# MathsionYang/Ransac

Hardware: NVIDIA B200
Metric: hypothesis x point evaluations/s (useful, whole job); ms per robust fit in config (higher is better)
Workload: dtype f32

## Files before the change

ransac_b200/csrc/common.cuh:

```cuda
#pragma once
#include <cuda_runtime.h>
#include <stdint.h>

#include "../../include/usac_gpu.h"

#define USAC_REC_STRIDE 32
#define USAC_TILE_PAIRS 128
#ifndef USAC_WARP_STAGES
#define USAC_WARP_STAGES 2
#endif
#define USAC_SCORE_THREADS 128
#ifndef USAC_SCORE_MIN_CTAS
#define USAC_SCORE_MIN_CTAS 4
#endif
#ifndef USAC_SCORE_GRID_CTAS
#define USAC_SCORE_GRID_CTAS USAC_SCORE_MIN_CTAS
#endif
#ifndef USAC_SQ_MIN_CTAS
#define USAC_SQ_MIN_CTAS 5
#endif
#ifndef USAC_PPI
#define USAC_PPI 4
#endif

enum { REC_MODEL = 0, REC_HINV = 9, REC_BAND = 18, REC_THR = 22 };

struct ProblemDesc {
    int n;
    int n_pairs;
    long long aos_off;
    long long pair_off;
    float mx1, my1, mx2, my2;
    int neigh_type, knn;
    long long knn_off;
    long long grid_off;
    long long cell_start_off;
    long long growth_off, term_off, pool_off;
    long long cursor_off;
};

struct FitState {
    float best_model[9];
    int best_cnt;
// ... 57 lines not shown
```

ransac_b200/csrc/pipeline.cuh:

```cuda
#pragma once
#include "strict_math.cuh"

struct RoundArgs {
    const ProblemDesc* prob;
    const int* active;
    FitState* state;
    const float* aos;
    int est, K, S, m, mstride;
    int e5_all_roots;
    int midx_shift;
    int sampler, rng, neighbors;
    uint64_t seed;
    const int* table; unsigned table_rows;
    const unsigned* growth;
    const int* knn; const int* cell_of_point; const int* members; const int* rank_in_cell; const int* cell_start;
    unsigned* cursors;
    int* seeds;
    int* samples;
    float* models_raw;
    int* nmodels;
    int* offsets;
    float* recs;
    int* mvalid;
    uint2* items;
    unsigned* item_count;
    int* part_cnt; float* part_sum; int nchunks;
    uint2* sample_scores;
    float thr, confidence;
    unsigned max_iterations;
    const unsigned* term_tables;
    int rank, nranks;
    int sprt;
    const int* pool;
    struct SprtModelResult* sprt_res;
    int* done_out;
    unsigned before_sprt;
    int limit_remaining;
    void* const* peer_win;
    void* peer_self;
    unsigned peer_seq;
    unsigned peer_cap;
    unsigned* peer_counter;
    int* peer_error;
    unsigned long long hyp_base_p1;
};

#define USAC_PEER_HEADER_BYTES 1024
#define USAC_PEER_MAX_RANKS 64
// ... 339 lines not shown
}

__global__ void __launch_bounds__(1024) prepare_kernel(const RoundArgs a) {
    __shared__ int sm[33];
    const int slot = blockIdx.x;
    const int pid = a.active[slot];
    const ProblemDesc pd = a.prob[pid];
    const int per = (a.K + blockDim.x - 1) / blockDim.x;
    const int j0 = threadIdx.x * per, j1 = min(j0 + per, a.K);
    const int* nm = a.nmodels + (size_t)slot * a.K;
    int local = 0;
    for (int j = j0; j < j1; j++) local += nm[j];
    int total;
    int off = block_exclusive_scan(local, &total, sm);
    float rec[USAC_REC_STRIDE];
    for (int j = j0; j < j1; j++) {
        a.offsets[(size_t)slot * a.K + j] = off;
        const int k = nm[j];
        for (int i = 0; i < k; i++) {
            make_record(a.est, a.models_raw + (((size_t)slot * a.K + j) * a.S + i) * 9, a.thr, pd, rec);
            float4* dst = reinterpret_cast<float4*>(a.recs + ((size_t)slot * a.mstride + off + i) * USAC_REC_STRIDE);
#pragma unroll
            for (int w = 0; w < USAC_REC_STRIDE / 4; w++) dst[w] = make_float4(rec[4 * w], rec[4 * w + 1], rec[4 * w + 2], rec[4 * w + 3]);
        }
        off += k;
    }
    if (threadIdx.x == 0) a.mvalid[slot] = total;
    if (a.items) {
        __shared__ unsigned s_base;
        const unsigned ngroups = (unsigned)(total + 31) / 32u, count = ngroups * (unsigned)a.nchunks;
        if (threadIdx.x == 0) s_base = atomicAdd(a.item_count, count);
        __syncthreads();
        for (unsigned i = threadIdx.x; i < count; i += blockDim.x)
            a.items[s_base + i] = make_uint2((unsigned)slot, ((i / ngroups) << 16) | (i % ngroups));
    }
}

__device__ __forceinline__ bool score_bigger(int ca, float sa, int cb, float sb) {
    return ca > cb || (ca == cb && sa > sb);
}
__device__ __forceinline__ unsigned pack_cnt_midx(const RoundArgs& a, int cnt, int midx) { return (unsigned)cnt | ((unsigned)midx << a.midx_shift); }
__device__ __forceinline__ int packed_cnt(const RoundArgs& a, unsigned x) { return (int)(x & ((1u << a.midx_shift) - 1u)); }
__device__ __forceinline__ int packed_midx(const RoundArgs& a, unsigned x) { return (int)(x >> a.midx_shift); }
__device__ __forceinline__ int midx_none(const RoundArgs& a) { return (int)(0xffffffffu >> a.midx_shift); }

__global__ void reduce_kernel(const RoundArgs a) {
    const int slot = blockIdx.y, j = blockIdx.x * blockDim.x + threadIdx.x;
    if (j < a.K && !(a.nranks > 1 && (j % a.nranks) != a.rank)) {
        const int k = a.nmodels[(size_t)slot * a.K + j];
        const int off = a.offsets[(size_t)slot * a.K + j];
        int bc = -1, bi = 0;
        float bs = 0.f;
        for (int i = 0; i < k; i++) {
            int c = 0;
            float s = 0.f;
            for (int ch = 0; ch < a.nchunks; ch++) {
                const size_t o = ((size_t)slot * a.nchunks + ch) * a.mstride + off + i;
// ... 191 lines not shown
```

ransac_b200/csrc/score.cuh:

```cuda
#pragma once
#include "strict_math.cuh"

__device__ __forceinline__ float fast_rcp(float x) { float r; asm("rcp.approx.ftz.f32 %0, %1;" : "=f"(r) : "f"(x)); return r; }
__device__ __forceinline__ float fast_sqrt(float x) { float r; asm("sqrt.approx.ftz.f32 %0, %1;" : "=f"(r) : "f"(x)); return r; }
__device__ __forceinline__ float fast_rsqrt(float x) { float r; asm("rsqrt.approx.ftz.f32 %0, %1;" : "=f"(r) : "f"(x)); return r; }
__device__ __forceinline__ float2 dup(float x) { return make_float2(x, x); }

__device__ __forceinline__ uint32_t smem_u32(const void* p) { return (uint32_t)__cvta_generic_to_shared(p); }
__device__ __forceinline__ void mbar_init(uint64_t* bar, uint32_t count) {
    asm volatile("mbarrier.init.shared::cta.b64 [%0], %1;" ::"r"(smem_u32(bar)), "r"(count));
}
__device__ __forceinline__ void mbar_expect_tx(uint64_t* bar, uint32_t bytes) {
    asm volatile("mbarrier.arrive.expect_tx.shared::cta.b64 _, [%0], %1;" ::"r"(smem_u32(bar)), "r"(bytes) : "memory");
}
__device__ __forceinline__ bool mbar_try_wait(uint64_t* bar, uint32_t parity) {
    uint32_t ok;
    asm volatile(
        "{\n\t.reg .pred p;\n\t"
        "mbarrier.try_wait.parity.shared::cta.b64 p, [%1], %2;\n\t"
        "selp.u32 %0, 1, 0, p;\n\t}"
        : "=r"(ok)
        : "r"(smem_u32(bar)), "r"(parity)
        : "memory");
    return ok != 0;
// ... 237 lines not shown
        return make_float2(fabsf(v.x) + (negthr - band), fabsf(v.y) + (negthr - band));
    }
    __device__ __forceinline__ float reject_bound() const { return 0.f; }
    static __device__ __forceinline__ float finish(float sum_em, int cnt, float thr) { return sum_em + (float)cnt * thr; }
    static __device__ __forceinline__ float strict_to_em(float err, float thr) { return err - thr; }
};

struct ScoreArgs {
    const float* pairs;
    const float* aos;
    const ProblemDesc* prob;
    const int* active;
    const float* recs;
    const int* mvalid;
    int M, mstride;
    int chunk_pairs, nchunks;
    int mblocks, slots;
    int* part_cnt;
    float* part_sum;
    unsigned* work;
    unsigned work_base;
    const uint2* items;
    const unsigned* item_count;
};

__device__ __forceinline__ bool score_item(const ScoreArgs& a, unsigned item, unsigned total, int mgroups, int& slot, int& chunk, int& mgroup) {
    if (item >= total) return false;
    if (a.items) {
        const uint2 it = a.items[item];
        slot = (int)it.x; chunk = (int)(it.y >> 16); mgroup = (int)(it.y & 0xffffu);
    } else {
        mgroup = (int)(item % (unsigned)mgroups);
        const unsigned rest = item / (unsigned)mgroups;
        chunk = (int)(rest % (unsigned)a.nchunks); slot = (int)(rest / (unsigned)a.nchunks);
    }
    return true;
}

template <int EST>
__device__ __noinline__ float strict_em(const float* __restrict__ rec, const float* __restrict__ aos, int idx, int n) {
    if (idx >= n) return 0.f;
    const float thr = rec[REC_THR];
    float err;
    if (EST == USAC_EST_LINE2D) {
        const float2 p = reinterpret_cast<const float2*>(aos)[idx];
        err = strict_error<EST>(rec, p.x, p.y, 0.f, 0.f);
    } else {
        const float4 p = reinterpret_cast<const float4*>(aos)[idx];
        err = strict_error<EST>(rec, p.x, p.y, p.z, p.w);
    }
    return (err < thr) ? FastModel<EST>::strict_to_em(err, thr) : 0.f;
}

template <int EST>
__global__ void __launch_bounds__(USAC_SCORE_THREADS, USAC_SCORE_MIN_CTAS) score_kernel(const ScoreArgs a) {
    constexpr int PAIR_FLOATS = (EST == USAC_EST_LINE2D) ? 4 : 8;
    constexpr int NWARPS = USAC_SCORE_THREADS / 32;
    __shared__ __align__(128) float tile_all[NWARPS][USAC_WARP_STAGES][USAC_TILE_PAIRS * PAIR_FLOATS];
    __shared__ __align__(8) uint64_t full_all[NWARPS][USAC_WARP_STAGES];

    const int lane = threadIdx.x & 31, warp = threadIdx.x >> 5;
    float (*tile)[USAC_TILE_PAIRS * PAIR_FLOATS] = tile_all[warp];
    uint64_t* full = full_all[warp];
    if (lane == 0) {
#pragma unroll
        for (int s = 0; s < USAC_WARP_STAGES; s++) mbar_init(&full[s], 1);
        asm volatile("fence.mbarrier_init.release.cluster;" ::: "memory");
        asm volatile("fence.proxy.async.shared::cta;" ::: "memory");
    }
    __syncwarp();

    const int mgroups = a.mblocks * NWARPS;
    const unsigned total = a.items ? *a.item_count : (unsigned)a.slots * (unsigned)a.nchunks * (unsigned)mgroups;
    uint32_t g = 0;

    for (;;) {
        unsigned item = 0;
        if (lane == 0) item = atomicAdd(a.work, 1u) - a.work_base;
        item = __shfl_sync(0xffffffffu, item, 0);
        int slot, chunk, mgroup;
        if (!score_item(a, item, total, mgroups, slot, chunk, mgroup)) break;
        const int M = a.mvalid ? a.mvalid[slot] : a.M;
        if (mgroup * 32 >= M) continue;
        const ProblemDesc pd = a.prob[a.active ? a.active[slot] : slot];
        const int m = mgroup * 32 + lane;
        const bool live = m < M;
        const float* rec = a.recs + ((size_t)slot * a.mstride + (live ? m : 0)) * USAC_REC_STRIDE;
        const size_t out = ((size_t)slot * a.nchunks + chunk) * a.mstride + m;

        const int pair_begin = chunk * a.chunk_pairs;
        const int npairs = min(pair_begin + a.chunk_pairs, pd.n_pairs) - pair_begin;
        if (npairs <= 0) {
            if (live) { a.part_cnt[out] = 0; a.part_sum[out] = 0.f; }
            continue;
        }
        const int ntiles = (npairs + USAC_TILE_PAIRS - 1) / USAC_TILE_PAIRS;
        const float* src = a.pairs + ((size_t)pd.pair_off + pair_begin) * PAIR_FLOATS;

        if (lane == 0) {
            asm volatile("fence.proxy.async.shared::cta;" ::: "memory");
            for (int k = 0; k < USAC_WARP_STAGES && k < ntiles; k++) {
                const int s = (g + k) % USAC_WARP_STAGES;
                const uint32_t bytes = min(USAC_TILE_PAIRS, npairs - k * USAC_TILE_PAIRS) * PAIR_FLOATS * 4;
                mbar_expect_tx(&full[s], bytes);
// ... 256 lines not shown
```

ransac_b200/csrc/score_sq.cuh:

```cuda
#pragma once
#include "score.cuh"

#ifndef USAC_SQ_TRIPVOTE
#define USAC_SQ_TRIPVOTE 2
#endif
#ifndef USAC_SQ_PREFETCH
#define USAC_SQ_PREFETCH 0
#endif
#define USAC_SQ_LANE_CAP 16
#define USAC_SQ_FIXED_BITS 36
#define USAC_SQ_LO_BITS 22

__device__ __forceinline__ void sq_push(bool pred, uint32_t& qaddr, uint32_t entry) {
    asm volatile(
        "{\n\t.reg .pred p;\n\t"
        "setp.ne.u32 p, %1, 0;\n\t"
        "@p st.shared.u32 [%0], %2;\n\t"
        "@p add.u32 %0, %0, 128;\n\t}"
        : "+r"(qaddr)
        : "r"((uint32_t)pred), "r"(entry));
}

template <int EST>
__device__ __noinline__ void sq_drain(const uint32_t* __restrict__ q, uint32_t cnt, uint32_t* pre, const float* __restrict__ recs_group,
                                      const float* __restrict__ aos, int n, double scale, uint32_t* mcnt, uint32_t* mlo, uint32_t* mhi) {
    const int lane = threadIdx.x & 31;
    uint32_t incl = cnt;
#pragma unroll
    for (int o = 1; o < 32; o <<= 1) { const uint32_t y = __shfl_up_sync(0xffffffffu, incl, o); if (lane >= o) incl += y; }
    const uint32_t total = __shfl_sync(0xffffffffu, incl, 31);
    pre[lane] = incl - cnt;
    __syncwarp();
    for (uint32_t base = 0; base < total; base += 64) {
        int l[2], idx[2];
        bool on[2];
        float4 p[2];
#pragma unroll
        for (int h = 0; h < 2; h++) {
            const uint32_t t = base + 32u * h + lane;
            on[h] = t < total;
            l[h] = 0; idx[h] = 0;
            if (on[h]) {
                int ll = 0;
#pragma unroll
                for (int step = 16; step; step >>= 1) if (pre[ll + step] <= t) ll += step;
                l[h] = ll;
                idx[h] = (int)q[(t - pre[ll]) * 32 + ll];
                on[h] = idx[h] < n;
            }
            p[h] = make_float4(0.f, 0.f, 0.f, 0.f);
            if (on[h]) {
                if (EST == USAC_EST_LINE2D) { const float2 v = reinterpret_cast<const float2*>(aos)[idx[h]]; p[h] = make_float4(v.x, v.y, 0.f, 0.f); }
                else p[h] = reinterpret_cast<const float4*>(aos)[idx[h]];
            }
        }
#pragma unroll
        for (int h = 0; h < 2; h++) {
            if (!on[h]) continue;
            const float* rec = recs_group + (size_t)l[h] * USAC_REC_STRIDE;
            const float err = strict_error<EST>(rec, p[h].x, p[h].y, p[h].z, p[h].w);
            if (err < rec[REC_THR]) {
                const unsigned long long fix = __double2ull_rn((double)err * scale);
                atomicAdd(&mcnt[l[h]], 1u);
                atomicAdd(&mlo[l[h]], (uint32_t)(fix & ((1u << USAC_SQ_LO_BITS) - 1u)));
                atomicAdd(&mhi[l[h]], (uint32_t)(fix >> USAC_SQ_LO_BITS));
            }
        }
    }
}

template <int EST>
__global__ void __launch_bounds__(USAC_SCORE_THREADS, USAC_SQ_MIN_CTAS) score_sq_kernel(const ScoreArgs a) {
    constexpr int PAIR_FLOATS = (EST == USAC_EST_LINE2D) ? 4 : 8;
    constexpr int NWARPS = USAC_SCORE_THREADS / 32;
    static_assert(USAC_SQ_LANE_CAP >= 4 * USAC_PPI, "a lane's queue must hold two trips of pushes");
    __shared__ __align__(128) float tile_all[NWARPS][USAC_WARP_STAGES][USAC_TILE_PAIRS * PAIR_FLOATS];
    __shared__ __align__(8) uint64_t full_all[NWARPS][USAC_WARP_STAGES];
    __shared__ __align__(128) uint32_t queue_all[NWARPS][USAC_SQ_LANE_CAP * 32];
    __shared__ uint32_t macc_all[NWARPS][4][32];

    const int lane = threadIdx.x & 31, warp = threadIdx.x >> 5;
    float (*tile)[USAC_TILE_PAIRS * PAIR_FLOATS] = tile_all[warp];
    uint64_t* full = full_all[warp];
    uint32_t* queue = queue_all[warp];
    uint32_t* mcnt = macc_all[warp][0];
    uint32_t* mlo = macc_all[warp][1];
    uint32_t* mhi = macc_all[warp][2];
    uint32_t* pre = macc_all[warp][3];
    const uint32_t q_first = smem_u32(queue) + 4u * (uint32_t)lane;
    const uint32_t q_limit = q_first + 128u * (USAC_SQ_LANE_CAP - 2 * USAC_PPI);
    if (lane == 0) {
#pragma unroll
        for (int s = 0; s < USAC_WARP_STAGES; s++) mbar_init(&full[s], 1);
        asm volatile("fence.mbarrier_init.release.cluster;" ::: "memory");
        asm volatile("fence.proxy.async.shared::cta;" ::: "memory");
    }
    __syncwarp();

    const int mgroups = a.mblocks * NWARPS;
    const unsigned total = a.items ? *a.item_count : (unsigned)a.slots * (unsigned)a.nchunks * (unsigned)mgroups;
    uint32_t g = 0;

    unsigned pending = 0;
    if (USAC_SQ_PREFETCH && lane == 0) pending = atomicAdd(a.work, 1u) - a.work_base;
    for (;;) {
        if (!USAC_SQ_PREFETCH && lane == 0) pending = atomicAdd(a.work, 1u) - a.work_base;
        const unsigned item = __shfl_sync(0xffffffffu, pending, 0);
        int slot, chunk, mgroup;
        if (!score_item(a, item, total, mgroups, slot, chunk, mgroup)) break;
        if (USAC_SQ_PREFETCH && lane == 0) pending = atomicAdd(a.work, 1u) - a.work_base;
        const int M = a.mvalid ? a.mvalid[slot] : a.M;
        if (mgroup * 32 >= M) continue;
        const ProblemDesc pd = a.prob[a.active ? a.active[slot] : slot];
        const int m = mgroup * 32 + lane;
        const bool live = m < M;
        const float* recs_group = a.recs + ((size_t)slot * a.mstride + (size_t)mgroup * 32) * USAC_REC_STRIDE;
        const float* rec = recs_group + (size_t)(live ? lane : 0) * USAC_REC_STRIDE;
        const size_t out = ((size_t)slot * a.nchunks + chunk) * a.mstride + m;

        const int pair_begin = chunk * a.chunk_pairs;
        const int npairs = min(pair_begin + a.chunk_pairs, pd.n_pairs) - pair_begin;
        if (npairs <= 0) {
            if (live) { a.part_cnt[out] = 0; a.part_sum[out] = 0.f; }
            continue;
        }
        const int ntiles = (npairs + USAC_TILE_PAIRS - 1) / USAC_TILE_PAIRS;
        const float* src = a.pairs + ((size_t)pd.pair_off + pair_begin) * PAIR_FLOATS;

        if (lane == 0) {
            asm volatile("fence.proxy.async.shared::cta;" ::: "memory");
            for (int k = 0; k < USAC_WARP_STAGES && k < ntiles; k++) {
                const int s = (g + k) % USAC_WARP_STAGES;
                const uint32_t bytes = min(USAC_TILE_PAIRS, npairs - k * USAC_TILE_PAIRS) * PAIR_FLOATS * 4;
                mbar_expect_tx(&full[s], bytes);
                bulk_copy_g2s(tile[s], src + (size_t)k * USAC_TILE_PAIRS * PAIR_FLOATS, bytes, &full[s]);
            }
        }
        mcnt[lane] = 0u; mlo[lane] = 0u; mhi[lane] = 0u;
        uint32_t acc_cnt = 0;
        unsigned long long acc_sum = 0;
        __syncwarp();

        FastModel<EST> fm;
        fm.load(rec);
        const float thr = rec[REC_THR];
        const double scale = (double)(1ull << USAC_SQ_FIXED_BITS) / (double)thr;
// ... 55 lines not shown
                        load_pair(j + q, A, B);
                        const float2 z = fm.reject(A, B);
                        sq_push(!(z.x > zb) && live, qaddr, ebase + 2 * q);
                        sq_push(!(z.y > zb) && live, qaddr, ebase + 2 * q + 1);
                    }
                }
                if (__any_sync(0xffffffffu, qaddr > q_limit)) drain();
            }
            __syncwarp();
            if (lane == 0 && k + USAC_WARP_STAGES < ntiles) {
                asm volatile("fence.proxy.async.shared::cta;" ::: "memory");
                const int nk = k + USAC_WARP_STAGES;
                const uint32_t bytes = min(USAC_TILE_PAIRS, npairs - nk * USAC_TILE_PAIRS) * PAIR_FLOATS * 4;
                mbar_expect_tx(&full[s], bytes);
                bulk_copy_g2s(tile[s], src + (size_t)nk * USAC_TILE_PAIRS * PAIR_FLOATS, bytes, &full[s]);
            }
        }
        g += (uint32_t)ntiles;
        if (__any_sync(0xffffffffu, qaddr != q_first)) drain();
        if (live) {
            a.part_cnt[out] = (int)acc_cnt;
            a.part_sum[out] = (float)((double)acc_sum / scale);
        }
        __syncwarp();
    }
}
```

ransac_b200/csrc/usac_gpu.cu:

```cuda
#include <dlfcn.h>

#include <cub/device/device_radix_sort.cuh>
#include <cub/device/device_scan.cuh>

#include <algorithm>
#include <chrono>
#include <cmath>
#include <cstdio>
#include <cstdlib>
#include <cstring>
#include <map>
#include <string>
#include <thread>
#include <tuple>
#include <vector>

#include "essential.cuh"
#include "pipeline.cuh"
#include "score.cuh"
#include "score_sq.cuh"
#include "sprt.cuh"
#include "refit.cuh"
#include "lo.cuh"
#include "knn.cuh"
// ... 67 lines not shown
    DevBuf<unsigned> d_sprt_count;
    cudaStream_t stream2 = nullptr;
    cudaEvent_t ev_block[2] = {nullptr, nullptr};
    cudaEvent_t ev_round = nullptr;
    DevBuf<int> d_lo_bwave;
    DevBuf<LoSpec> d_lo_spec;
    DevBuf<LoWaveState> d_lo_ws;
    PinnedBuf<LoWaveState> h_lo_ws;
    DevBuf<unsigned> d_inl_ballots;
    DevBuf<int> d_inl_counts;
    PinnedBuf<int> h_rp_nmodels;
    PinnedBuf<SprtModelResult> h_rp_res;
    PinnedBuf<int2> h_rp_scores;
    PinnedBuf<float> h_rp_models;
    PinnedBuf<FitState> h_rp_state;
    DevBuf<int2> d_model_scores;
    DevBuf<float> d_pool_pts;
    DevBuf<unsigned long long> d_grid_keys;
    DevBuf<int> d_grid_ints;
    DevBuf<unsigned char> d_grid_temp;
    DevBuf<unsigned> d_work;
    DevBuf<uint2> d_items;
    DevBuf<unsigned> d_item_count;
    unsigned work_next = 0;
    DevBuf<int> d_knn_cells;
    DevBuf<float4> d_knn_pts;
    DevBuf<float> d_q_models, d_q_recs, d_q_sum, d_q_err;
    DevBuf<int> d_q_cnt, d_q_ids, d_q_ids2, d_q_ok, d_lo_ids_a, d_lo_ids_b, d_lo_small;
    DevBuf<float> d_q_model2;
    DevBuf<LoIO> d_lo_io;
    usac_allgather_fn allgather = nullptr;
    void* allgather_user = nullptr;
    void* nccl_lib = nullptr;
    void* nccl_comm = nullptr;
    void* peer_self = nullptr;
    unsigned peer_cap = 0;
    std::vector<void*> peer_opened;
    DevBuf<void*> d_peer_win;
    DevBuf<unsigned> d_peer_counter;
    DevBuf<int> d_peer_error;
    int* h_peer_error = nullptr;
    int peer_rank = -1, peer_nranks = 0;
    unsigned peer_seq = 0;
    unsigned long long peer_rounds = 0;
    std::map<std::tuple<int, int, float, unsigned>, std::vector<unsigned>> term_cache;
    std::vector<long long> term_signature;
// ... 68 lines not shown
}

extern "C" void usac_gpu_destroy(usac_gpu_ctx* c) {
    if (!c) return;
    cudaSetDevice(c->device);
    cudaStreamSynchronize(c->stream);
    if (c->stream2) cudaStreamDestroy(c->stream2);
    for (int i = 0; i < 2; i++) if (c->ev_block[i]) cudaEventDestroy(c->ev_block[i]);
    if (c->ev_round) cudaEventDestroy(c->ev_round);
    for (void* w : c->peer_opened) cudaIpcCloseMemHandle(w);
    if (c->peer_self) cudaFree(c->peer_self);
    if (c->h_peer_error) cudaFreeHost(c->h_peer_error);
    c->d_peer_win.release(); c->d_peer_counter.release(); c->d_peer_error.release();
    if (c->nccl_comm && c->nccl_lib) {
        typedef int (*destroy_fn)(void*);
        destroy_fn f = (destroy_fn)dlsym(c->nccl_lib, "ncclCommDestroy");
        if (f) f(c->nccl_comm);
    }
    c->d_aos.release(); c->d_pairs.release(); c->d_prob.release(); c->d_pair_offs.release(); c->d_state.release(); c->d_active.release(); c->d_active2.release(); c->d_state_init.release();
    c->d_knn.release(); c->d_cell_of_point.release(); c->d_members.release(); c->d_rank.release(); c->d_cell_start.release();
    c->d_pool.release(); c->d_cursors.release(); c->d_growth.release(); c->d_term.release();
    c->d_samples.release(); c->d_nmodels.release(); c->d_offsets.release(); c->d_mvalid.release(); c->d_part_cnt.release();
    c->d_seeds.release(); c->d_table.release(); c->d_models_raw.release(); c->d_recs.release(); c->d_part_sum.release();
    c->d_scores.release(); c->d_scores_all.release(); c->d_sprt_res.release(); c->d_sprt_carry.release(); c->d_sprt_count.release(); c->d_inl_ballots.release(); c->d_inl_counts.release(); c->d_lo_bwave.release(); c->d_lo_spec.release(); c->d_lo_ws.release(); c->h_lo_ws.release(); c->h_rp_nmodels.release(); c->h_rp_res.release(); c->h_rp_scores.release(); c->h_rp_models.release(); c->h_rp_state.release(); c->d_model_scores.release(); c->d_pool_pts.release(); c->d_grid_keys.release(); c->d_grid_ints.release(); c->d_grid_temp.release(); c->d_knn_cells.release(); c->d_knn_pts.release(); c->d_work.release(); c->d_items.release(); c->d_item_count.release();
    c->d_q_models.release(); c->d_q_recs.release(); c->d_q_sum.release(); c->d_q_err.release(); c->d_q_cnt.release(); c->d_q_ids.release(); c->d_q_ids2.release(); c->d_q_ok.release(); c->d_q_model2.release(); c->d_lo_ids_a.release(); c->d_lo_ids_b.release(); c->d_lo_small.release(); c->d_lo_io.release();
    if (c->h_state) cudaFreeHost(c->h_state);
    if (c->h_active) cudaFreeHost(c->h_active);
    if (c->h_done) cudaFreeHost(c->h_done);
    c->d_done.release();
    for (auto& pr : c->score_events) { cudaEventDestroy(pr.first); cudaEventDestroy(pr.second); }
    cudaEventDestroy(c->ev0); cudaEventDestroy(c->ev1);
    if (c->own_stream) cudaStreamDestroy(c->stream);
    delete c;
}

extern "C" int usac_gpu_set_stream(usac_gpu_ctx* c, void* cuda_stream) {
    if (!c) return USAC_ERR_ARG;
    cudaSetDevice(c->device);
    CUDA_TRY(c, cudaStreamSynchronize(c->stream));
    if (c->own_stream) cudaStreamDestroy(c->stream);
    c->stream = (cudaStream_t)cuda_stream;
    c->own_stream = false;
    return USAC_OK;
}

extern "C" const char* usac_gpu_last_error(const usac_gpu_ctx* c) { return c ? c->err.c_str() : g_create_error.c_str(); }

// ... 360 lines not shown
    u.grid += (size_t)n;
    u.cell_start += (size_t)n + 1;
    if (d.cursor_off < 0) CUDA_TRY(c, append_segment(c->d_cursors, u.cursors, (const unsigned*)nullptr, 3 * (size_t)n + 1, &d.cursor_off, c->stream));
    d.neigh_type = USAC_NEIGH_GRID;
    return push_desc(c);
}

extern "C" int usac_gpu_set_sprt_pool(usac_gpu_ctx* c, int problem, const int* pool) {
    if (!c || problem < 0 || problem >= c->P || !pool) return fail(c, USAC_ERR_ARG, "set_sprt_pool: bad arguments");
    cudaSetDevice(c->device);
    SideUsed& u = c->side;
    ProblemDesc& d = c->h_prob[problem];
    for (int i = 0; i < d.n; i++) if (pool[i] < 0 || pool[i] >= d.n) return fail(c, USAC_ERR_ARG, "set_sprt_pool: index out of range");
    CUDA_TRY(c, append_segment(c->d_pool, u.pool, pool, (size_t)d.n, &d.pool_off, c->stream));
    const int dim = usac_point_dim(c->est);
    CUDA_TRY(c, c->d_pool_pts.ensure((size_t)c->total_points * dim));
    pool_gather_kernel<<<(d.n + 255) / 256, 256, 0, c->stream>>>(c->d_aos.p + (size_t)d.aos_off * dim, c->d_pool.p + d.pool_off, d.n, dim,
                                                                  c->d_pool_pts.p + (size_t)d.aos_off * dim);
    CUDA_TRY(c, cudaGetLastError());
    c->h_pool_set[problem] = 1;
    return push_desc(c);
}

static void launch_score(usac_gpu_ctx* c, ScoreArgs a, int slots, int mblocks, bool dense_survivors = false) {
    a.mblocks = mblocks; a.slots = slots;
    constexpr int warps_per_cta = USAC_SCORE_THREADS / 32;
    const long long items = (long long)slots * a.nchunks * mblocks * warps_per_cta;
    const unsigned grid = (unsigned)std::min<long long>((items + warps_per_cta - 1) / warps_per_cta,
                                                        (long long)c->prop.multiProcessorCount * USAC_SCORE_GRID_CTAS);
    static const int legacy = [] { const char* e = getenv("USAC_GPU_SCORE_LEGACY"); return e ? atoi(e) : 0; }();
    const bool loop_kernel = legacy == 1 || c->est == USAC_EST_LINE2D || (dense_survivors && legacy != 2);
    unsigned grid_ctas = grid;
    if (a.items) {
        grid_ctas = (unsigned)c->prop.multiProcessorCount * (loop_kernel ? USAC_SCORE_GRID_CTAS : USAC_SQ_MIN_CTAS);
        a.work = c->d_item_count.p + 1; a.work_base = 0;
    } else {
        if (!loop_kernel) grid_ctas = (unsigned)std::min<long long>((items + warps_per_cta - 1) / warps_per_cta, (long long)c->prop.multiProcessorCount * USAC_SQ_MIN_CTAS);
        a.work = c->d_work.p; a.work_base = c->work_next;
        c->work_next += (unsigned)items + grid_ctas * warps_per_cta;
    }
    auto& ev = c->next_score_event();
    cudaEventRecord(ev.first, c->stream);
    if (loop_kernel) {
        switch (c->est) {
            case USAC_EST_LINE2D: score_kernel<USAC_EST_LINE2D><<<grid_ctas, USAC_SCORE_THREADS, 0, c->stream>>>(a); break;
            case USAC_EST_HOMOGRAPHY: score_kernel<USAC_EST_HOMOGRAPHY><<<grid_ctas, USAC_SCORE_THREADS, 0, c->stream>>>(a); break;
            case USAC_EST_FUNDAMENTAL: score_kernel<USAC_EST_FUNDAMENTAL><<<grid_ctas, USAC_SCORE_THREADS, 0, c->stream>>>(a); break;
            default: score_kernel<USAC_EST_ESSENTIAL><<<grid_ctas, USAC_SCORE_THREADS, 0, c->stream>>>(a); break;
        }
    } else {
        switch (c->est) {
            case USAC_EST_HOMOGRAPHY: score_sq_kernel<USAC_EST_HOMOGRAPHY><<<grid_ctas, USAC_SCORE_THREADS, 0, c->stream>>>(a); break;
            case USAC_EST_FUNDAMENTAL: score_sq_kernel<USAC_EST_FUNDAMENTAL><<<grid_ctas, USAC_SCORE_THREADS, 0, c->stream>>>(a); break;
            default: score_sq_kernel<USAC_EST_ESSENTIAL><<<grid_ctas, USAC_SCORE_THREADS, 0, c->stream>>>(a); break;
// ... 232 lines not shown
        launch_nonminimal(c, aos, cur, best, c->d_q_model2.p, c->d_q_ok.p);
        prepare_models_kernel<<<1, 32, 0, c->stream>>>(c->est, c->d_q_model2.p, 1, w, threshold, c->d_prob.p, problem, c->d_q_recs.p);
        rc = launch_inliers(c, aos, d.n, c->d_q_recs.p, threshold, alt, alt + d.n);
        if (rc) return rc;
        c->last_launches++;
        CUDA_TRY(c, cudaMemcpyAsync(m2, c->d_q_model2.p, sizeof(float) * w, cudaMemcpyDeviceToHost, c->stream));
        CUDA_TRY(c, cudaMemcpyAsync(&ok, c->d_q_ok.p, sizeof(int), cudaMemcpyDeviceToHost, c->stream));
        CUDA_TRY(c, cudaMemcpyAsync(&c2, alt + d.n, sizeof(int), cudaMemcpyDeviceToHost, c->stream));
        CUDA_TRY(c, cudaStreamSynchronize(c->stream));
        CUDA_TRY(c, cudaGetLastError());
        if (!ok) break;
        if ((float)c2 / best < 0.8f) break;
        if ((unsigned)c2 <= (unsigned)prev) break;
        prev = c2; best = c2;
        std::swap(cur, alt);
        for (int i = 0; i < w; i++) out->model[i] = m2[i];
        out->accepted++;
    }
    out->inliers = best;
    return USAC_OK;
}

static void standard_termination_table(unsigned n, int m, float confidence, unsigned max_iterations, std::vector<unsigned>& out) {
    out.resize((size_t)n + 2);
    const float log_1_p = (float)logf(1 - confidence);
    auto fill = [&](unsigned lo, unsigned hi) {
        for (unsigned inl = lo; inl < hi; inl++) out[inl] = standard_termination_value(inl, n, m, log_1_p, max_iterations);
    };
    const unsigned total = n + 1;
    unsigned nthreads = total >= (1u << 16) ? std::min(16u, std::max(1u, std::thread::hardware_concurrency())) : 1u;
    if (nthreads <= 1) fill(0, total);
    else {
        std::vector<std::thread> pool;
        const unsigned per = (total + nthreads - 1) / nthreads;
        for (unsigned t = 0; t < nthreads; t++) pool.emplace_back(fill, std::min(total, t * per), std::min(total, (t + 1) * per));
        for (auto& th : pool) th.join();
    }
    unsigned peak = 0;
    for (unsigned inl = 0; inl < total; inl++) peak = std::max(peak, out[inl]);
    out[total] = peak;
}

static void prosac_growth(unsigned n, unsigned m, std::vector<unsigned>& g) {
    g.resize(n);
    double T_n = 200000;
    for (unsigned i = 0; i < m; ++i) T_n *= (double)(m - i) / (n - i);
    unsigned T_n_prime = 1;
    for (unsigned i = 0; i < n; ++i) {
        if (i + 1 <= m) { g[i] = T_n_prime; continue; }
        double Tn_plus1 = (double)(i + 1) * T_n / (i + 1 - m);
        g[i] = T_n_prime + (unsigned)ceil(Tn_plus1 - T_n);
        T_n = Tn_plus1;
        T_n_prime = g[i];
    }
}

static int fit_models_per_sample(int est, const usac_fit_cfg* cfg) {
    return cfg->essential_roots == USAC_E5_ROOTS_ALL_VALID ? USAC_E5_MAX_ROOTS : usac_models_per_sample(est);
}

static int ensure_round_buffers(usac_gpu_ctx* c, int slots, int K, int nchunks, int nranks, int S) {
    const int m = usac_sample_size(c->est);
    const size_t sk = (size_t)slots * K;
    CUDA_TRY(c, c->d_samples.ensure(sk * m));
    CUDA_TRY(c, c->d_nmodels.ensure(sk));
    CUDA_TRY(c, c->d_offsets.ensure(sk));
    CUDA_TRY(c, c->d_mvalid.ensure((size_t)slots + 1));
    CUDA_TRY(c, c->d_models_raw.ensure(sk * S * 9));
    CUDA_TRY(c, c->d_recs.ensure(sk * S * USAC_REC_STRIDE));
    CUDA_TRY(c, c->d_part_cnt.ensure(sk * S * nchunks));
    CUDA_TRY(c, c->d_part_sum.ensure(sk * S * nchunks));
    CUDA_TRY(c, c->d_seeds.ensure(sk));
    const size_t per_rank = (K + nranks - 1) / nranks;
    CUDA_TRY(c, c->d_scores.ensure(std::max(sk, (size_t)slots * per_rank)));
    CUDA_TRY(c, c->d_scores_all.ensure((size_t)slots * per_rank * nranks));
    CUDA_TRY(c, c->d_sprt_res.ensure(sk * S));
    CUDA_TRY(c, c->d_items.ensure((size_t)slots * nchunks * ((size_t)(K * S + 31) / 32)));
    CUDA_TRY(c, c->d_item_count.ensure(2));
    return USAC_OK;
}

static int setup_sampler_side(usac_gpu_ctx* c, const usac_sampler_cfg& s, bool reset_cursors = true) {
    if (s.sampler == USAC_SAMPLER_PROSAC) {
        std::vector<unsigned> all, g;
        for (int p = 0; p < c->P; p++) {
            prosac_growth((unsigned)c->h_prob[p].n, (unsigned)usac_sample_size(c->est), g);
            c->h_prob[p].growth_off = (long long)all.size();
            all.insert(all.end(), g.begin(), g.end());
        }
        CUDA_TRY(c, c->d_growth.ensure(all.size()));
        CUDA_TRY(c, cudaMemcpyAsync(c->d_growth.p, all.data(), sizeof(unsigned) * all.size(), cudaMemcpyHostToDevice, c->stream));
        CUDA_TRY(c, cudaStreamSynchronize(c->stream));
    }
    if (s.sampler == USAC_SAMPLER_NAPSAC) {
        for (int p = 0; p < c->P; p++) {
            const ProblemDesc& d = c->h_prob[p];
            if (s.neighbors == USAC_NEIGH_KNN ? d.knn_off < 0 : d.grid_off < 0) return fail(c, USAC_ERR_STATE, "NAPSAC: neighbourhood of a problem was not set");
            if (reset_cursors) {
                CUDA_TRY(c, cudaMemsetAsync(c->d_cursors.p + d.cursor_off, 0, sizeof(unsigned) * d.n, c->stream));
                CUDA_TRY(c, cudaMemsetAsync(c->d_cursors.p + d.cursor_off + 3 * (size_t)d.n, 0xFF, sizeof(unsigned), c->stream));
            }
// ... 930 lines not shown
    cudaEventRecord(c->ev0, c->stream);

    const char* growth_env = getenv("USAC_GPU_ROUND_GROWTH");
    const int growth_cap = growth_env ? atoi(growth_env) : 8;
    const bool k_free = growth_cap > 1 && !cfg->sprt && cfg->sampler.sampler != USAC_SAMPLER_PROSAC && cfg->sampler.rng != USAC_RNG_TABLE;
    const int K0 = K;
    const auto t_setup = now();
    while (!active.empty()) {
        const auto t_r0 = now();
        const int slots = (int)active.size();
        if (k_free && slots < P) {
            long long kr = std::min<long long>({2048LL, (long long)P * K0 / slots, (long long)K0 * growth_cap});
            kr = std::min<long long>(kr, std::max(cfg->max_iterations, 1u));
            kr = std::max<long long>(K0, kr / 128 * 128);
            if (nranks > 1) kr = (kr + nranks - 1) / nranks * nranks;
            K = (int)kr;
        }
        int max_pairs = 0;
        for (int p : active) max_pairs = std::max(max_pairs, c->h_prob[p].n_pairs);
        const int mblocks = (K * S + USAC_SCORE_THREADS - 1) / USAC_SCORE_THREADS;
        int chunk_pairs, nchunks;
        const int expect_models = (c->est == USAC_EST_FUNDAMENTAL || c->est == USAC_EST_ESSENTIAL) ? (K + 1) / 2 : K;
        plan_chunks(c, slots, std::max(1, ((expect_models + USAC_SCORE_THREADS - 1) / USAC_SCORE_THREADS) / nranks), max_pairs, &chunk_pairs, &nchunks);
        rc = ensure_round_buffers(c, slots, K, nchunks, nranks, S);
        if (rc) return rc;
        RoundArgs a;
        fill_round_args(c, a, cfg->sampler, K, S);
        a.active = act_cur;
        a.thr = cfg->threshold; a.confidence = cfg->confidence; a.max_iterations = cfg->max_iterations;
        a.table_rows = cfg->sample_table_rows; a.rank = rank; a.nranks = nranks; a.nchunks = nchunks;
        a.sprt = cfg->sprt; a.pool = c->d_pool.p; a.sprt_res = c->d_sprt_res.p; a.done_out = c->d_done.p;
        a.limit_remaining = 1;
        a.items = c->d_items.p; a.item_count = c->d_item_count.p;
        const bool use_peer = nranks > 1 && peers_ready && (size_t)nranks * slots * ((K + nranks - 1) / nranks) <= c->peer_cap;
        if (nranks > 1 && !use_peer && !c->allgather) return fail(c, USAC_ERR_STATE, "fit: the round does not fit the peer windows and no all-gather hook is installed");
        if (use_peer) {
            a.peer_win = c->d_peer_win.p; a.peer_self = c->peer_self; a.peer_cap = c->peer_cap;
            a.peer_counter = c->d_peer_counter.p; a.peer_error = c->d_peer_error.p;
        }
        int rounds_ahead = 1;
        if (P == 1 && max_n >= 65536) rounds_ahead = (int)std::min<unsigned>(8u, (cfg->max_iterations + (unsigned)K - 1) / (unsigned)K);
        for (int ahead = 0; ahead < rounds_ahead; ahead++) {
            TK("round");
            CUDA_TRY(c, cudaMemsetAsync(c->d_item_count.p, 0, 2 * sizeof(unsigned), c->stream));

            launch_sampler(c, a, slots);
            TK("sampler");
            switch (c->est) {
                case USAC_EST_LINE2D: launch_round_est<USAC_EST_LINE2D>(c, a, slots, cfg->sprt); break;
                case USAC_EST_HOMOGRAPHY: launch_round_est<USAC_EST_HOMOGRAPHY>(c, a, slots, cfg->sprt); break;
                case USAC_EST_FUNDAMENTAL: launch_round_est<USAC_EST_FUNDAMENTAL>(c, a, slots, cfg->sprt); break;
                default: launch_round_est<USAC_EST_ESSENTIAL>(c, a, slots, cfg->sprt); break;
            }
            TK("solve");
            prepare_kernel<<<slots, (slots == 1 && K >= 1024) ? 1024 : 256, 0, c->stream>>>(a);
            c->last_launches++;
            {
                ScoreArgs sa{};
                sa.pairs = c->d_pairs.p; sa.aos = c->d_aos.p; sa.prob = c->d_prob.p; sa.active = act_cur; sa.recs = c->d_recs.p;
                sa.mvalid = c->d_mvalid.p; sa.M = K * S; sa.mstride = K * S; sa.chunk_pairs = chunk_pairs; sa.nchunks = nchunks;
                sa.part_cnt = c->d_part_cnt.p; sa.part_sum = c->d_part_sum.p;
                sa.items = c->d_items.p; sa.item_count = c->d_item_count.p;
                TK("prepare");
                launch_score(c, sa, slots, mblocks);
                TK("score");
                dim3 gr((K + 127) / 128, slots);
                if (use_peer) { a.peer_seq = ++c->peer_seq; c->peer_rounds++; }
                const dim3 grc_grid(((K + nranks - 1) / nranks + 31) / 32, slots);
                if (nchunks > 8 && S > 3) reduce_chunks_kernel<USAC_E5_MAX_ROOTS><<<grc_grid, 256, 0, c->stream>>>(a);
                else if (nchunks > 8) reduce_chunks_kernel<USAC_MAX_MODELS_PER_SAMPLE><<<grc_grid, 256, 0, c->stream>>>(a);
                else reduce_kernel<<<gr, 128, 0, c->stream>>>(a);
                c->last_launches++;
                const uint2* scores = c->d_scores.p;
                TK("reduce");
                if (nranks > 1 && !use_peer) {
                    const size_t bytes = (size_t)slots * (K / nranks) * sizeof(uint2);
                    int grc = c->allgather(c->allgather_user, c->d_scores.p, c->d_scores_all.p, bytes, (void*)c->stream);
                    if (grc) return fail(c, USAC_ERR_NCCL, "fit: all-gather failed");
                    scores = c->d_scores_all.p;
                }
                TK("allgather");
                select_kernel<<<slots, 256, 0, c->stream>>>(a, scores);
                c->last_launches++;
            }
            switch (c->est) {
// ... 230 lines not shown
```

Before: 1089 billion.

## Skip scoring of hypotheses past an early-termination cutoff within a round

Work items are reordered into bands by model group so earlier samples get scored first across all slots. As each model group finishes all chunks, its inlier count is looked up in a suffix-max termination table to lower a per-slot sample cutoff. Later groups whose sample index lies beyond that cutoff write zero partial scores and skip the scan. This adds atomics, extra buffers, a last-block scan in prepare and a band search in the work loop, and it changes which hypotheses get fully evaluated.

```diff
diff --git a/ransac_b200/csrc/common.cuh b/ransac_b200/csrc/common.cuh
--- a/ransac_b200/csrc/common.cuh
+++ b/ransac_b200/csrc/common.cuh
@@ -19,6 +19,10 @@
 #ifndef USAC_SQ_MIN_CTAS
 #define USAC_SQ_MIN_CTAS 5
 #endif
+#ifndef USAC_CUT_BAND_GROUPS
+#define USAC_CUT_BAND_GROUPS 2
+#endif
+#define USAC_MAX_BANDS 256
 #ifndef USAC_PPI
 #define USAC_PPI 4
 #endif
diff --git a/ransac_b200/csrc/pipeline.cuh b/ransac_b200/csrc/pipeline.cuh
--- a/ransac_b200/csrc/pipeline.cuh
+++ b/ransac_b200/csrc/pipeline.cuh
@@ -24,6 +24,12 @@
     int* mvalid;
     uint2* items;
     unsigned* item_count;
+    int band_groups, nbands;
+    unsigned band_cap;
+    unsigned* cut;
+    int* msample;
+    unsigned* mtot;
+    unsigned* grp_done;
     int* part_cnt; float* part_sum; int nchunks;
     uint2* sample_scores;
     float thr, confidence;
@@ -409,17 +415,49 @@
             float4* dst = reinterpret_cast<float4*>(a.recs + ((size_t)slot * a.mstride + off + i) * USAC_REC_STRIDE);
 #pragma unroll
             for (int w = 0; w < USAC_REC_STRIDE / 4; w++) dst[w] = make_float4(rec[4 * w], rec[4 * w + 1], rec[4 * w + 2], rec[4 * w + 3]);
+            if (a.cut) a.msample[(size_t)slot * a.mstride + off + i] = j;
         }
         off += k;
     }
     if (threadIdx.x == 0) a.mvalid[slot] = total;
+    const unsigned ngroups = (unsigned)(total + 31) / 32u;
+    if (a.cut) {
+        const FitState& st = a.state[pid];
+        for (int i = threadIdx.x; i < total; i += blockDim.x) a.mtot[(size_t)slot * a.mstride + i] = 0u;
+        for (unsigned i = threadIdx.x; i < ngroups; i += blockDim.x) a.grp_done[(size_t)slot * ((a.mstride + 31) / 32) + i] = 0u;
+        if (threadIdx.x == 0) {
+            const unsigned reach = samples_in_reach(a, pd, st);
+            a.cut[2 * slot] = reach <= st.iters ? 0u : min((unsigned)a.K, reach - st.iters);
+            a.cut[2 * slot + 1] = st.iters;
+        }
+    }
     if (a.items) {
-        __shared__ unsigned s_base;
-        const unsigned ngroups = (unsigned)(total + 31) / 32u, count = ngroups * (unsigned)a.nchunks;
-        if (threadIdx.x == 0) s_base = atomicAdd(a.item_count, count);
+        __shared__ unsigned s_base[USAC_MAX_BANDS];
+        __shared__ int s_last;
+        const unsigned G = (unsigned)a.band_groups, per_band = G * (unsigned)a.nchunks;
+        const unsigned nb = (ngroups + G - 1) / G, count = ngroups * (unsigned)a.nchunks;
+        unsigned* band_count = a.item_count + 3;
+        for (unsigned b = threadIdx.x; b < nb; b += blockDim.x)
+            s_base[b] = b * a.band_cap + atomicAdd(band_count + b, (min(ngroups, (b + 1) * G) - b * G) * (unsigned)a.nchunks);
         __syncthreads();
-        for (unsigned i = threadIdx.x; i < count; i += blockDim.x)
-            a.items[s_base + i] = make_uint2((unsigned)slot, ((i / ngroups) << 16) | (i % ngroups));
+        for (unsigned i = threadIdx.x; i < count; i += blockDim.x) {
+            const unsigned b = i / per_band, r = i - b * per_band, gb = min(ngroups, (b + 1) * G) - b * G;
+            a.items[s_base[b] + r] = make_uint2((unsigned)slot, ((r / gb) << 16) | (b * G + r % gb));
+        }
+        __threadfence();
+        __syncthreads();
+        if (threadIdx.x == 0) s_last = atomicAdd(a.item_count + 2, 1u) == gridDim.x - 1;
+        __syncthreads();
+        if (s_last) {
+            __threadfence();
+            const int b = threadIdx.x;
+            const int v = b < a.nbands ? (int)__ldcg(band_count + b) : 0;
+            int all;
+            const int start = block_exclusive_scan(v, &all, sm);
+            unsigned* band_start = band_count + a.nbands;
+            if (b < a.nbands) band_start[b] = (unsigned)start;
+            if (b == 0) { band_start[a.nbands] = (unsigned)all; a.item_count[0] = (unsigned)all; }
+        }
     }
 }
 
diff --git a/ransac_b200/csrc/score.cuh b/ransac_b200/csrc/score.cuh
--- a/ransac_b200/csrc/score.cuh
+++ b/ransac_b200/csrc/score.cuh
@@ -283,12 +283,21 @@
     unsigned work_base;
     const uint2* items;
     const unsigned* item_count;
+    const unsigned* band_start;
+    int nbands;
+    unsigned band_cap;
+    unsigned* cut;
+    const int* msample;
+    unsigned* mtot;
+    unsigned* grp_done;
+    const unsigned* term_tables;
 };
 
-__device__ __forceinline__ bool score_item(const ScoreArgs& a, unsigned item, unsigned total, int mgroups, int& slot, int& chunk, int& mgroup) {
+__device__ __forceinline__ bool score_item(const ScoreArgs& a, unsigned item, unsigned total, int mgroups, int& slot, int& chunk, int& mgroup, int& band) {
     if (item >= total) return false;
     if (a.items) {
-        const uint2 it = a.items[item];
+        while (band + 1 < a.nbands && a.band_start[band + 1] <= item) band++;
+        const uint2 it = a.items[(size_t)band * a.band_cap + (item - a.band_start[band])];
         slot = (int)it.x; chunk = (int)(it.y >> 16); mgroup = (int)(it.y & 0xffffu);
     } else {
         mgroup = (int)(item % (unsigned)mgroups);
@@ -334,13 +343,14 @@
     const int mgroups = a.mblocks * NWARPS;
     const unsigned total = a.items ? *a.item_count : (unsigned)a.slots * (unsigned)a.nchunks * (unsigned)mgroups;
     uint32_t g = 0;
+    int band = 0;
 
     for (;;) {
         unsigned item = 0;
         if (lane == 0) item = atomicAdd(a.work, 1u) - a.work_base;
         item = __shfl_sync(0xffffffffu, item, 0);
         int slot, chunk, mgroup;
-        if (!score_item(a, item, total, mgroups, slot, chunk, mgroup)) break;
+        if (!score_item(a, item, total, mgroups, slot, chunk, mgroup, band)) break;
         const int M = a.mvalid ? a.mvalid[slot] : a.M;
         if (mgroup * 32 >= M) continue;
         const ProblemDesc pd = a.prob[a.active ? a.active[slot] : slot];
diff --git a/ransac_b200/csrc/score_sq.cuh b/ransac_b200/csrc/score_sq.cuh
--- a/ransac_b200/csrc/score_sq.cuh
+++ b/ransac_b200/csrc/score_sq.cuh
@@ -21,6 +21,12 @@
         : "r"((uint32_t)pred), "r"(entry));
 }
 
+__device__ __forceinline__ unsigned ld_relaxed_u32(const unsigned* p) {
+    unsigned v;
+    asm volatile("ld.relaxed.gpu.global.u32 %0, [%1];" : "=r"(v) : "l"(p) : "memory");
+    return v;
+}
+
 template <int EST>
 __device__ __noinline__ void sq_drain(const uint32_t* __restrict__ q, uint32_t cnt, uint32_t* pre, const float* __restrict__ recs_group,
                                       const float* __restrict__ aos, int n, double scale, uint32_t* mcnt, uint32_t* mlo, uint32_t* mhi) {
@@ -67,6 +73,31 @@
             }
         }
     }
+}
+
+__device__ __noinline__ void sq_item_done(const ScoreArgs& a, int slot, int mgroup, bool live, uint32_t cnt) {
+    const int lane = threadIdx.x & 31;
+    const size_t mi = (size_t)slot * a.mstride + (size_t)mgroup * 32 + (live ? lane : 0);
+    const ProblemDesc& pd = a.prob[a.active ? a.active[slot] : slot];
+    if (live && cnt) atomicAdd(a.mtot + mi, cnt);
+    __syncwarp();
+    unsigned last = 0;
+    if (lane == 0) {
+        unsigned done;
+        asm volatile("atom.acq_rel.gpu.global.add.u32 %0, [%1], 1;" : "=r"(done) : "l"(a.grp_done + (size_t)slot * ((a.mstride + 31) / 32) + mgroup) : "memory");
+        last = done == (unsigned)a.nchunks - 1u;
+    }
+    if (!__shfl_sync(0xffffffffu, last, 0)) return;
+    unsigned bound = 0xffffffffu;
+    if (live) {
+        const unsigned c = __ldcg(a.mtot + mi);
+        const unsigned R = a.term_tables[pd.term_off + (size_t)pd.n + 2 + c];
+        const unsigned iters0 = a.cut[2 * slot + 1];
+        bound = max((unsigned)a.msample[mi] + 1u, R > iters0 ? R - iters0 : 0u);
+    }
+#pragma unroll
+    for (int o = 16; o; o >>= 1) bound = min(bound, __shfl_xor_sync(0xffffffffu, bound, o));
+    if (lane == 0) atomicMin(a.cut + 2 * slot, bound);
 }
 
 template <int EST>
@@ -100,6 +131,7 @@
     const int mgroups = a.mblocks * NWARPS;
     const unsigned total = a.items ? *a.item_count : (unsigned)a.slots * (unsigned)a.nchunks * (unsigned)mgroups;
     uint32_t g = 0;
+    int band = 0;
 
     unsigned pending = 0;
     if (USAC_SQ_PREFETCH && lane == 0) pending = atomicAdd(a.work, 1u) - a.work_base;
@@ -107,21 +139,30 @@
         if (!USAC_SQ_PREFETCH && lane == 0) pending = atomicAdd(a.work, 1u) - a.work_base;
         const unsigned item = __shfl_sync(0xffffffffu, pending, 0);
         int slot, chunk, mgroup;
-        if (!score_item(a, item, total, mgroups, slot, chunk, mgroup)) break;
+        if (!score_item(a, item, total, mgroups, slot, chunk, mgroup, band)) break;
         if (USAC_SQ_PREFETCH && lane == 0) pending = atomicAdd(a.work, 1u) - a.work_base;
         const int M = a.mvalid ? a.mvalid[slot] : a.M;
         if (mgroup * 32 >= M) continue;
-        const ProblemDesc pd = a.prob[a.active ? a.active[slot] : slot];
         const int m = mgroup * 32 + lane;
         const bool live = m < M;
+        const size_t out = ((size_t)slot * a.nchunks + chunk) * a.mstride + m;
+        if (a.cut) {
+            unsigned past = 0;
+            if (lane == 0) past = (unsigned)a.msample[(size_t)slot * a.mstride + (size_t)mgroup * 32] >= ld_relaxed_u32(a.cut + 2 * slot);
+            if (__shfl_sync(0xffffffffu, past, 0)) {
+                if (live) { a.part_cnt[out] = 0; a.part_sum[out] = 0.f; }
+                continue;
+            }
+        }
+        const ProblemDesc pd = a.prob[a.active ? a.active[slot] : slot];
         const float* recs_group = a.recs + ((size_t)slot * a.mstride + (size_t)mgroup * 32) * USAC_REC_STRIDE;
         const float* rec = recs_group + (size_t)(live ? lane : 0) * USAC_REC_STRIDE;
-        const size_t out = ((size_t)slot * a.nchunks + chunk) * a.mstride + m;
 
         const int pair_begin = chunk * a.chunk_pairs;
         const int npairs = min(pair_begin + a.chunk_pairs, pd.n_pairs) - pair_begin;
         if (npairs <= 0) {
             if (live) { a.part_cnt[out] = 0; a.part_sum[out] = 0.f; }
+            if (a.cut) sq_item_done(a, slot, mgroup, live, 0u);
             continue;
         }
         const int ntiles = (npairs + USAC_TILE_PAIRS - 1) / USAC_TILE_PAIRS;
@@ -223,6 +264,7 @@
             a.part_cnt[out] = (int)acc_cnt;
             a.part_sum[out] = (float)((double)acc_sum / scale);
         }
+        if (a.cut) sq_item_done(a, slot, mgroup, live, acc_cnt);
         __syncwarp();
     }
 }
diff --git a/ransac_b200/csrc/usac_gpu.cu b/ransac_b200/csrc/usac_gpu.cu
--- a/ransac_b200/csrc/usac_gpu.cu
+++ b/ransac_b200/csrc/usac_gpu.cu
@@ -113,6 +113,8 @@
     DevBuf<unsigned> d_work;
     DevBuf<uint2> d_items;
     DevBuf<unsigned> d_item_count;
+    DevBuf<unsigned> d_cut, d_mtot, d_grp_done;
+    DevBuf<int> d_msample;
     unsigned work_next = 0;
     DevBuf<int> d_knn_cells;
     DevBuf<float4> d_knn_pts;
@@ -227,7 +229,7 @@
     c->d_pool.release(); c->d_cursors.release(); c->d_growth.release(); c->d_term.release();
     c->d_samples.release(); c->d_nmodels.release(); c->d_offsets.release(); c->d_mvalid.release(); c->d_part_cnt.release();
     c->d_seeds.release(); c->d_table.release(); c->d_models_raw.release(); c->d_recs.release(); c->d_part_sum.release();
-    c->d_scores.release(); c->d_scores_all.release(); c->d_sprt_res.release(); c->d_sprt_carry.release(); c->d_sprt_count.release(); c->d_inl_ballots.release(); c->d_inl_counts.release(); c->d_lo_bwave.release(); c->d_lo_spec.release(); c->d_lo_ws.release(); c->h_lo_ws.release(); c->h_rp_nmodels.release(); c->h_rp_res.release(); c->h_rp_scores.release(); c->h_rp_models.release(); c->h_rp_state.release(); c->d_model_scores.release(); c->d_pool_pts.release(); c->d_grid_keys.release(); c->d_grid_ints.release(); c->d_grid_temp.release(); c->d_knn_cells.release(); c->d_knn_pts.release(); c->d_work.release(); c->d_items.release(); c->d_item_count.release();
+    c->d_scores.release(); c->d_scores_all.release(); c->d_sprt_res.release(); c->d_sprt_carry.release(); c->d_sprt_count.release(); c->d_inl_ballots.release(); c->d_inl_counts.release(); c->d_lo_bwave.release(); c->d_lo_spec.release(); c->d_lo_ws.release(); c->h_lo_ws.release(); c->h_rp_nmodels.release(); c->h_rp_res.release(); c->h_rp_scores.release(); c->h_rp_models.release(); c->h_rp_state.release(); c->d_model_scores.release(); c->d_pool_pts.release(); c->d_grid_keys.release(); c->d_grid_ints.release(); c->d_grid_temp.release(); c->d_knn_cells.release(); c->d_knn_pts.release(); c->d_work.release(); c->d_items.release(); c->d_item_count.release(); c->d_cut.release(); c->d_mtot.release(); c->d_grp_done.release(); c->d_msample.release();
     c->d_q_models.release(); c->d_q_recs.release(); c->d_q_sum.release(); c->d_q_err.release(); c->d_q_cnt.release(); c->d_q_ids.release(); c->d_q_ids2.release(); c->d_q_ok.release(); c->d_q_model2.release(); c->d_lo_ids_a.release(); c->d_lo_ids_b.release(); c->d_lo_small.release(); c->d_lo_io.release();
     if (c->h_state) cudaFreeHost(c->h_state);
     if (c->h_active) cudaFreeHost(c->h_active);
@@ -634,14 +636,18 @@
     return push_desc(c);
 }
 
+static bool score_loop_kernel(const usac_gpu_ctx* c, bool dense_survivors) {
+    static const int legacy = [] { const char* e = getenv("USAC_GPU_SCORE_LEGACY"); return e ? atoi(e) : 0; }();
+    return legacy == 1 || c->est == USAC_EST_LINE2D || (dense_survivors && legacy != 2);
+}
+
 static void launch_score(usac_gpu_ctx* c, ScoreArgs a, int slots, int mblocks, bool dense_survivors = false) {
     a.mblocks = mblocks; a.slots = slots;
     constexpr int warps_per_cta = USAC_SCORE_THREADS / 32;
     const long long items = (long long)slots * a.nchunks * mblocks * warps_per_cta;
     const unsigned grid = (unsigned)std::min<long long>((items + warps_per_cta - 1) / warps_per_cta,
                                                         (long long)c->prop.multiProcessorCount * USAC_SCORE_GRID_CTAS);
-    static const int legacy = [] { const char* e = getenv("USAC_GPU_SCORE_LEGACY"); return e ? atoi(e) : 0; }();
-    const bool loop_kernel = legacy == 1 || c->est == USAC_EST_LINE2D || (dense_survivors && legacy != 2);
+    const bool loop_kernel = score_loop_kernel(c, dense_survivors);
     unsigned grid_ctas = grid;
     if (a.items) {
         grid_ctas = (unsigned)c->prop.multiProcessorCount * (loop_kernel ? USAC_SCORE_GRID_CTAS : USAC_SQ_MIN_CTAS);
@@ -920,7 +926,7 @@
 }
 
 static void standard_termination_table(unsigned n, int m, float confidence, unsigned max_iterations, std::vector<unsigned>& out) {
-    out.resize((size_t)n + 2);
+    out.resize(2 * (size_t)n + 3);
     const float log_1_p = (float)logf(1 - confidence);
     auto fill = [&](unsigned lo, unsigned hi) {
         for (unsigned inl = lo; inl < hi; inl++) out[inl] = standard_termination_value(inl, n, m, log_1_p, max_iterations);
@@ -937,6 +943,8 @@
     unsigned peak = 0;
     for (unsigned inl = 0; inl < total; inl++) peak = std::max(peak, out[inl]);
     out[total] = peak;
+    unsigned run = 0;
+    for (unsigned inl = total; inl-- > 0;) { run = std::max(run, out[inl]); out[total + 1 + inl] = run; }
 }
 
 static void prosac_growth(unsigned n, unsigned m, std::vector<unsigned>& g) {
@@ -957,7 +965,7 @@
     return cfg->essential_roots == USAC_E5_ROOTS_ALL_VALID ? USAC_E5_MAX_ROOTS : usac_models_per_sample(est);
 }
 
-static int ensure_round_buffers(usac_gpu_ctx* c, int slots, int K, int nchunks, int nranks, int S) {
+static int ensure_round_buffers(usac_gpu_ctx* c, int slots, int K, int nchunks, int nranks, int S, int nbands = 1, size_t band_cap = 0, bool cut = false) {
     const int m = usac_sample_size(c->est);
     const size_t sk = (size_t)slots * K;
     CUDA_TRY(c, c->d_samples.ensure(sk * m));
@@ -973,8 +981,14 @@
     CUDA_TRY(c, c->d_scores.ensure(std::max(sk, (size_t)slots * per_rank)));
     CUDA_TRY(c, c->d_scores_all.ensure((size_t)slots * per_rank * nranks));
     CUDA_TRY(c, c->d_sprt_res.ensure(sk * S));
-    CUDA_TRY(c, c->d_items.ensure((size_t)slots * nchunks * ((size_t)(K * S + 31) / 32)));
-    CUDA_TRY(c, c->d_item_count.ensure(2));
+    CUDA_TRY(c, c->d_items.ensure(std::max((size_t)nbands * band_cap, (size_t)slots * nchunks * ((size_t)(K * S + 31) / 32))));
+    CUDA_TRY(c, c->d_item_count.ensure(4 + 2 * (size_t)nbands));
+    if (cut) {
+        CUDA_TRY(c, c->d_cut.ensure(2 * (size_t)slots));
+        CUDA_TRY(c, c->d_msample.ensure(sk * S));
+        CUDA_TRY(c, c->d_mtot.ensure(sk * S));
+        CUDA_TRY(c, c->d_grp_done.ensure((size_t)slots * ((size_t)(K * S + 31) / 32)));
+    }
     return USAC_OK;
 }
 
@@ -1951,7 +1965,12 @@
         int chunk_pairs, nchunks;
         const int expect_models = (c->est == USAC_EST_FUNDAMENTAL || c->est == USAC_EST_ESSENTIAL) ? (K + 1) / 2 : K;
         plan_chunks(c, slots, std::max(1, ((expect_models + USAC_SCORE_THREADS - 1) / USAC_SCORE_THREADS) / nranks), max_pairs, &chunk_pairs, &nchunks);
-        rc = ensure_round_buffers(c, slots, K, nchunks, nranks, S);
+        const bool cut = nranks == 1 && !score_loop_kernel(c, false);
+        const int groups = (K * S + 31) / 32;
+        const int band_groups = cut ? std::max(USAC_CUT_BAND_GROUPS, (groups + USAC_MAX_BANDS - 1) / USAC_MAX_BANDS) : groups;
+        const int nbands = (groups + band_groups - 1) / band_groups;
+        const size_t band_cap = (size_t)slots * band_groups * nchunks;
+        rc = ensure_round_buffers(c, slots, K, nchunks, nranks, S, nbands, band_cap, cut);
         if (rc) return rc;
         RoundArgs a;
         fill_round_args(c, a, cfg->sampler, K, S);
@@ -1961,6 +1980,8 @@
         a.sprt = cfg->sprt; a.pool = c->d_pool.p; a.sprt_res = c->d_sprt_res.p; a.done_out = c->d_done.p;
         a.limit_remaining = 1;
         a.items = c->d_items.p; a.item_count = c->d_item_count.p;
+        a.band_groups = band_groups; a.nbands = nbands; a.band_cap = (unsigned)band_cap;
+        if (cut) { a.cut = c->d_cut.p; a.msample = c->d_msample.p; a.mtot = c->d_mtot.p; a.grp_done = c->d_grp_done.p; }
         const bool use_peer = nranks > 1 && peers_ready && (size_t)nranks * slots * ((K + nranks - 1) / nranks) <= c->peer_cap;
         if (nranks > 1 && !use_peer && !c->allgather) return fail(c, USAC_ERR_STATE, "fit: the round does not fit the peer windows and no all-gather hook is installed");
         if (use_peer) {
@@ -1971,7 +1992,7 @@
         if (P == 1 && max_n >= 65536) rounds_ahead = (int)std::min<unsigned>(8u, (cfg->max_iterations + (unsigned)K - 1) / (unsigned)K);
         for (int ahead = 0; ahead < rounds_ahead; ahead++) {
             TK("round");
-            CUDA_TRY(c, cudaMemsetAsync(c->d_item_count.p, 0, 2 * sizeof(unsigned), c->stream));
+            CUDA_TRY(c, cudaMemsetAsync(c->d_item_count.p, 0, (4 + 2 * (size_t)nbands) * sizeof(unsigned), c->stream));
 
             launch_sampler(c, a, slots);
             TK("sampler");
@@ -1990,6 +2011,9 @@
                 sa.mvalid = c->d_mvalid.p; sa.M = K * S; sa.mstride = K * S; sa.chunk_pairs = chunk_pairs; sa.nchunks = nchunks;
                 sa.part_cnt = c->d_part_cnt.p; sa.part_sum = c->d_part_sum.p;
                 sa.items = c->d_items.p; sa.item_count = c->d_item_count.p;
+                sa.band_start = c->d_item_count.p + 3 + nbands; sa.nbands = nbands; sa.band_cap = (unsigned)band_cap;
+                sa.cut = a.cut; sa.msample = a.msample; sa.mtot = a.mtot; sa.grp_done = a.grp_done;
+                sa.term_tables = c->d_term.p;
                 TK("prepare");
                 launch_score(c, sa, slots, mblocks);
                 TK("score");
```

After: 1136 billion, median of 6. +4.4%, better.
